# smpurkis/PyTorch-Face-Detection-from-Scratch

Measured on AMD Instinct MI355X. Metric: train imgs/sec (PoolResnet 480^2, bs=256 per GPU), higher is better.
Workload: dtype f32 (3x3 convs: bf16x3 split MFMA, fp32 accumulate)

## Files before the change

pytorch-face-detection-from-scratch_amd/csrc/fdet_ps.hip:

```cpp
#include "fdet_ps.h"

using namespace fdet;

namespace {

__global__ void __launch_bounds__(256)
k_ps_from_f32(const float* __restrict__ x, ps_bf16x8* __restrict__ ps, PsGeo g, PsStrips st, int total) {
  const int t = blockIdx.x * 256 + threadIdx.x;
  if (t >= total) return;
  const int xx = t % st.Wf, r = t / st.Wf;
  const int y = r % g.H, r2 = r / g.H;
  const int gr = r2 % g.C8, n = r2 / g.C8;
  const size_t HW = (size_t)g.H * st.Wf;
  const float* src = x + ((size_t)n * g.C + gr * 8) * HW + (size_t)y * st.Wf + xx;
  ps_bf16x8 hi, lo;
#pragma unroll
  for (int j = 0; j < 8; ++j) {
    const float f = src[j * HW];
    const __bf16 h = (__bf16)f;
    hi[j] = h;
    lo[j] = (__bf16)(f - (float)h);
  }
  const int sidx = xx / st.Ws, xs = xx - sidx * st.Ws;
  const size_t u = (size_t)(sidx * st.Nimg + n) * g.img + (size_t)(gr * g.HP + y) * g.WP + xs + 1;
  ps[u] = hi;
  ps[u + g.plane] = lo;
  if (xs == 0 && sidx > 0) {
    const size_t v = u - (size_t)st.Nimg * g.img + st.Ws;
    ps[v] = hi;
    ps[v + g.plane] = lo;
  }
  if (xs == st.Ws - 1 && sidx + 1 < st.S) {
    const size_t v = u + (size_t)st.Nimg * g.img - st.Ws;
    ps[v] = hi;
    ps[v + g.plane] = lo;
  }
}

__global__ void __launch_bounds__(256)
k_ps_halo(ps_bf16x8* __restrict__ ps, PsGeo g, PsStrips st, int planes, int mode, int total) {
  const int t = blockIdx.x * 256 + threadIdx.x;
  if (t >= total) return;
  const int y = t % g.H;
  int r = t / g.H;
  const int gr = r % g.C8; r /= g.C8;
  const int pl = r % planes; r /= planes;
  const int n = r % st.Nimg, e = r / st.Nimg;
  const size_t row = (size_t)pl * g.plane + (size_t)(gr * g.HP + y) * g.WP;
  const size_t left = (size_t)(e * st.Nimg + n) * g.img + row, right = left + (size_t)st.Nimg * g.img;
  if (mode == 0) {
    ps[left + st.Ws + 1] = ps[right + 1];
    ps[right] = ps[left + st.Ws];
  } else {
    const ps_bf16x8 z = {};
    ps[left + st.Ws + 1] = z;
    ps[right] = z;
  }
}

__global__ void __launch_bounds__(256)
k_ps_to_f32(const ps_bf16x8* __restrict__ ps, float* __restrict__ x, PsGeo g, PsStrips st, int total) {
  const int t = blockIdx.x * 256 + threadIdx.x;
  if (t >= total) return;
  const int xx = t % st.Wf, r = t / st.Wf;
  const int y = r % g.H, r2 = r / g.H;
  const int gr = r2 % g.C8, n = r2 / g.C8;
  const size_t HW = (size_t)g.H * st.Wf;
  const int sidx = xx / st.Ws, xs = xx - sidx * st.Ws;
  const size_t u = (size_t)(sidx * st.Nimg + n) * g.img + (size_t)(gr * g.HP + y) * g.WP + xs + 1;
  const ps_bf16x8 hi = ps[u], lo = ps[u + g.plane];
  float* dst = x + ((size_t)n * g.C + gr * 8) * HW + (size_t)y * st.Wf + xx;
#pragma unroll
  for (int j = 0; j < 8; ++j) dst[j * HW] = (float)hi[j] + (float)lo[j];
}

template <bool P16>
__global__ void __launch_bounds__(256)
k_pool_route_bwd_ps(const float* __restrict__ dout, const unsigned char* __restrict__ route8, const float* __restrict__ scale,
                    ps_bf16x8* __restrict__ dz, PsGeo g, PsStrips st, int Hp, int Wp, float slope, int total) {
  const int t = blockIdx.x * 256 + threadIdx.x;
  if (t >= total) return;
  const int xg = t % Wp, r = t / Wp;
  const int yp = r % Hp, r2 = r / Hp;
  const int gr = r2 % g.C8, n = r2 / g.C8;
  const size_t HWp = (size_t)Hp * Wp;
  const float* src = dout + ((size_t)n * g.C + gr * 8) * HWp + (size_t)yp * Wp + xg;
  const int wsp = st.Ws >> 1, sidx = xg / wsp, xp = xg - sidx * wsp, ns = sidx * st.Nimg + n;
  typedef unsigned u32x2 __attribute__((ext_vector_type(2)));
  const u32x2 rb = *reinterpret_cast<const u32x2*>(route8 + (((size_t)(ns * g.C8 + gr) * Hp + yp) * (g.W >> 1) + xp) * 8);
  float gv[8];
  unsigned mk[8];
#pragma unroll
  for (int j = 0; j < 8; ++j) {
    gv[j] = src[j * HWp] * (scale ? scale[n * g.C + gr * 8 + j] : 1.f);
    mk[j] = (rb[j >> 2] >> (8 * (j & 3))) & 0xffu;
  }
#pragma unroll
  for (int k = 0; k < 4; ++k) {
    ps_bf16x8 hi, lo;
#pragma unroll
    for (int j = 0; j < 8; ++j) {
      const float f = ((int)((mk[j] >> 4) & 3) == k) ? gv[j] * (((mk[j] >> k) & 1) ? 1.f : slope) : 0.f;
      const __bf16 h = (__bf16)f;
      hi[j] = h;
      if (!P16) lo[j] = (__bf16)(f - (float)h);
    }
    const size_t u = (size_t)ns * g.img + (size_t)(gr * g.HP + 2 * yp + (k >> 1)) * g.WP + 2 * xp + (k & 1) + 1;
    dz[u] = hi;
    if (!P16) dz[u + g.plane] = lo;
  }
  if (st.S > 1) {
    const ps_bf16x8 zero = {};
    const bool left = xp == 0 && sidx > 0, right = xp == wsp - 1 && sidx + 1 < st.S;
    if (left || right) {
#pragma unroll
      for (int rr = 0; rr < 2; ++rr) {
        const size_t row = (size_t)ns * g.img + (size_t)(gr * g.HP + 2 * yp + rr) * g.WP;
        if (left) { dz[row] = zero; if (!P16) dz[row + g.plane] = zero; }
        if (right) { dz[row + st.Ws + 1] = zero; if (!P16) dz[row + st.Ws + 1 + g.plane] = zero; }
      }
    }
  }
}

}

namespace {
int pool_route_bwd_ps_run(const float* dout_pooled, const unsigned char* route8, const float* drop_scale,
                          void* dz2_ps, int N, int C, int H, int W, float slope, void* stream, bool p16) {
  PsGeo g;
  PsStrips sp;
  FDET_REQUIRE(dout_pooled && route8 && dz2_ps && !(H & 1) && !(W & 1) && ps_geo_strips(N, C, H, W, g, sp),
               "pool_route_bwd_ps: unsupported shape N=%d C=%d H=%d W=%d (even H, W; C %% 8 == 0)", N, C, H, W);
  const long long total = (long long)N * g.C8 * (H / 2) * (W / 2);
  FDET_REQUIRE(total < (1ll << 31), "pool_route_bwd_ps: tensor too large");
  if (p16)
    hipLaunchKernelGGL(k_pool_route_bwd_ps<true>, dim3((unsigned)((total + 255) / 256)), dim3(256), 0, (hipStream_t)stream,
                       dout_pooled, route8, drop_scale, reinterpret_cast<ps_bf16x8*>(dz2_ps), g, sp, H / 2, W / 2, slope, (int)total);
  else
    hipLaunchKernelGGL(k_pool_route_bwd_ps<false>, dim3((unsigned)((total + 255) / 256)), dim3(256), 0, (hipStream_t)stream,
                       dout_pooled, route8, drop_scale, reinterpret_cast<ps_bf16x8*>(dz2_ps), g, sp, H / 2, W / 2, slope, (int)total);
  return check_launch("fdet_pool_route_bwd_ps");
}
}

extern "C" int fdet_pool_route_bwd_ps(const float* dout_pooled, const unsigned char* route8, const float* drop_scale,
                                      void* dz2_ps, int N, int C, int H, int W, float slope, void* stream) {
  return pool_route_bwd_ps_run(dout_pooled, route8, drop_scale, dz2_ps, N, C, H, W, slope, stream, false);
}
extern "C" int fdet_pool_route_bwd_ps_p16(const float* dout_pooled, const unsigned char* route8, const float* drop_scale,
                                          void* dz2_ps, int N, int C, int H, int W, float slope, void* stream) {
  return pool_route_bwd_ps_run(dout_pooled, route8, drop_scale, dz2_ps, N, C, H, W, slope, stream, true);
}

extern "C" size_t fdet_ps_bytes(int N, int C, int H, int W) {
  PsGeo g;
  PsStrips sp;
  if (!ps_geo_strips(N, C, H, W, g, sp)) return 0;
  return (size_t)(g.N + 2) * g.img * 16;
}

extern "C" size_t fdet_ps_image0_offset(int N, int C, int H, int W) {
  PsGeo g;
  PsStrips sp;
  if (!ps_geo_strips(N, C, H, W, g, sp)) return 0;
  return (size_t)g.img * 16;
}

extern "C" int fdet_ps_strips(int W) {
  PsGeo g;
  PsStrips sp;
  return ps_geo_strips(1, 8, 2, W, g, sp) ? sp.S : 0;
}

extern "C" int fdet_ps_halo_exchange(void* ps, int N, int C, int H, int W, int zero_only, int hi_only, void* stream) {
  PsGeo g;
  PsStrips sp;
  FDET_REQUIRE(ps && ps_geo_strips(N, C, H, W, g, sp), "ps_halo_exchange: unsupported shape N=%d C=%d H=%d W=%d", N, C, H, W);
  if (sp.S == 1) return FDET_OK;
  const int planes = hi_only ? 1 : 2;
  const long long total = (long long)(sp.S - 1) * N * planes * g.C8 * H;
  FDET_REQUIRE(total < (1ll << 31), "ps_halo_exchange: tensor too large");
  hipLaunchKernelGGL(k_ps_halo, dim3((unsigned)((total + 255) / 256)), dim3(256), 0, (hipStream_t)stream,
                     reinterpret_cast<ps_bf16x8*>(ps), g, sp, planes, zero_only ? 1 : 0, (int)total);
  return check_launch("fdet_ps_halo_exchange");
}

extern "C" int fdet_ps_from_f32(const float* x, void* ps, int N, int C, int H, int W, void* stream) {
  PsGeo g;
  PsStrips sp;
  FDET_REQUIRE(x && ps && ps_geo_strips(N, C, H, W, g, sp), "ps_from_f32: unsupported shape N=%d C=%d H=%d W=%d", N, C, H, W);
  const long long total = (long long)N * g.C8 * H * W;
  FDET_REQUIRE(total < (1ll << 31), "ps_from_f32: tensor too large");
  hipLaunchKernelGGL(k_ps_from_f32, dim3((unsigned)((total + 255) / 256)), dim3(256), 0, (hipStream_t)stream, x,
                     reinterpret_cast<ps_bf16x8*>(ps), g, sp, (int)total);
  return check_launch("fdet_ps_from_f32");
}

extern "C" int fdet_ps_to_f32(const void* ps, float* x, int N, int C, int H, int W, void* stream) {
  PsGeo g;
  PsStrips sp;
  FDET_REQUIRE(x && ps && ps_geo_strips(N, C, H, W, g, sp), "ps_to_f32: unsupported shape N=%d C=%d H=%d W=%d", N, C, H, W);
  const long long total = (long long)N * g.C8 * H * W;
  FDET_REQUIRE(total < (1ll << 31), "ps_to_f32: tensor too large");
  hipLaunchKernelGGL(k_ps_to_f32, dim3((unsigned)((total + 255) / 256)), dim3(256), 0, (hipStream_t)stream,
                     reinterpret_cast<const ps_bf16x8*>(ps), x, g, sp, (int)total);
  return check_launch("fdet_ps_to_f32");
}
```

Baseline: 91520.

## Remap pool-route backward to one wavefront per padded output row

```diff
diff --git a/pytorch-face-detection-from-scratch_amd/csrc/fdet_ps.hip b/pytorch-face-detection-from-scratch_amd/csrc/fdet_ps.hip
--- a/pytorch-face-detection-from-scratch_amd/csrc/fdet_ps.hip
+++ b/pytorch-face-detection-from-scratch_amd/csrc/fdet_ps.hip
@@ -74,18 +74,21 @@
   for (int j = 0; j < 8; ++j) dst[j * HW] = (float)hi[j] + (float)lo[j];
 }
 
-template <bool P16>
+template <int WPT, bool P16>
 __global__ void __launch_bounds__(256)
 k_pool_route_bwd_ps(const float* __restrict__ dout, const unsigned char* __restrict__ route8, const float* __restrict__ scale,
-                    ps_bf16x8* __restrict__ dz, PsGeo g, PsStrips st, int Hp, int Wp, float slope, int total) {
-  const int t = blockIdx.x * 256 + threadIdx.x;
-  if (t >= total) return;
-  const int xg = t % Wp, r = t / Wp;
-  const int yp = r % Hp, r2 = r / Hp;
-  const int gr = r2 % g.C8, n = r2 / g.C8;
+                    ps_bf16x8* __restrict__ dz, PsGeo g, PsStrips st, int Hp, int Wp, float slope, int rows) {
+  const int lane = threadIdx.x & 63;
+  const int row = __builtin_amdgcn_readfirstlane((int)(blockIdx.x * 4 + (threadIdx.x >> 6)));
+  if (row >= rows || (WPT == 16 && lane >= 32)) return;
+  const int yp = row % Hp, r2 = row / Hp;
+  const int gr = r2 % g.C8, ns = r2 / g.C8;
+  const int sidx = ns / st.Nimg, n = ns - sidx * st.Nimg;
+  const int s = lane & (WPT - 1), x = s - 1;
+  const bool real = s >= 1 && s <= (sidx == st.S - 1 ? st.Wlast : st.Ws);
+  const int xp = real ? x >> 1 : 0, cp = x & 1;
   const size_t HWp = (size_t)Hp * Wp;
-  const float* src = dout + ((size_t)n * g.C + gr * 8) * HWp + (size_t)yp * Wp + xg;
-  const int wsp = st.Ws >> 1, sidx = xg / wsp, xp = xg - sidx * wsp, ns = sidx * st.Nimg + n;
+  const float* src = dout + ((size_t)n * g.C + gr * 8) * HWp + (size_t)yp * Wp + sidx * (st.Ws >> 1) + xp;
   typedef unsigned u32x2 __attribute__((ext_vector_type(2)));
   const u32x2 rb = *reinterpret_cast<const u32x2*>(route8 + (((size_t)(ns * g.C8 + gr) * Hp + yp) * (g.W >> 1) + xp) * 8);
   float gv[8];
@@ -96,50 +99,53 @@
     mk[j] = (rb[j >> 2] >> (8 * (j & 3))) & 0xffu;
   }
 #pragma unroll
-  for (int k = 0; k < 4; ++k) {
-    ps_bf16x8 hi, lo;
-#pragma unroll
-    for (int j = 0; j < 8; ++j) {
-      const float f = ((int)((mk[j] >> 4) & 3) == k) ? gv[j] * (((mk[j] >> k) & 1) ? 1.f : slope) : 0.f;
-      const __bf16 h = (__bf16)f;
-      hi[j] = h;
-      if (!P16) lo[j] = (__bf16)(f - (float)h);
+  for (int rr = 0; rr < (WPT == 64 ? 2 : 1); ++rr) {
+    const int r = WPT == 64 ? rr : lane / WPT, k = 2 * r + cp;
+    ps_bf16x8 hi = {}, lo = {};
+    if (real) {
+#pragma unroll
+      for (int j = 0; j < 8; ++j) {
+        const float f = ((int)((mk[j] >> 4) & 3) == k) ? gv[j] * (((mk[j] >> k) & 1) ? 1.f : slope) : 0.f;
+        const __bf16 h = (__bf16)f;
+        hi[j] = h;
+        if (!P16) lo[j] = (__bf16)(f - (float)h);
+      }
     }
-    const size_t u = (size_t)ns * g.img + (size_t)(gr * g.HP + 2 * yp + (k >> 1)) * g.WP + 2 * xp + (k & 1) + 1;
+    const size_t u = (size_t)ns * g.img + (size_t)(gr * g.HP + 2 * yp + r) * g.WP + s;
     dz[u] = hi;
     if (!P16) dz[u + g.plane] = lo;
   }
-  if (st.S > 1) {
-    const ps_bf16x8 zero = {};
-    const bool left = xp == 0 && sidx > 0, right = xp == wsp - 1 && sidx + 1 < st.S;
-    if (left || right) {
-#pragma unroll
-      for (int rr = 0; rr < 2; ++rr) {
-        const size_t row = (size_t)ns * g.img + (size_t)(gr * g.HP + 2 * yp + rr) * g.WP;
-        if (left) { dz[row] = zero; if (!P16) dz[row + g.plane] = zero; }
-        if (right) { dz[row + st.Ws + 1] = zero; if (!P16) dz[row + st.Ws + 1 + g.plane] = zero; }
-      }
-    }
-  }
 }
 
 }
 
 namespace {
+template <int WPT>
+void pool_route_bwd_ps_launch(const float* dout_pooled, const unsigned char* route8, const float* drop_scale, void* dz2_ps,
+                              const PsGeo& g, const PsStrips& sp, int Hp, int Wp, float slope, int rows, void* stream, bool p16) {
+  const dim3 grid((unsigned)((rows + 3) / 4));
+  if (p16)
+    hipLaunchKernelGGL((k_pool_route_bwd_ps<WPT, true>), grid, dim3(256), 0, (hipStream_t)stream,
+                       dout_pooled, route8, drop_scale, reinterpret_cast<ps_bf16x8*>(dz2_ps), g, sp, Hp, Wp, slope, rows);
+  else
+    hipLaunchKernelGGL((k_pool_route_bwd_ps<WPT, false>), grid, dim3(256), 0, (hipStream_t)stream,
+                       dout_pooled, route8, drop_scale, reinterpret_cast<ps_bf16x8*>(dz2_ps), g, sp, Hp, Wp, slope, rows);
+}
+
 int pool_route_bwd_ps_run(const float* dout_pooled, const unsigned char* route8, const float* drop_scale,
                           void* dz2_ps, int N, int C, int H, int W, float slope, void* stream, bool p16) {
   PsGeo g;
   PsStrips sp;
   FDET_REQUIRE(dout_pooled && route8 && dz2_ps && !(H & 1) && !(W & 1) && ps_geo_strips(N, C, H, W, g, sp),
                "pool_route_bwd_ps: unsupported shape N=%d C=%d H=%d W=%d (even H, W; C %% 8 == 0)", N, C, H, W);
-  const long long total = (long long)N * g.C8 * (H / 2) * (W / 2);
-  FDET_REQUIRE(total < (1ll << 31), "pool_route_bwd_ps: tensor too large");
-  if (p16)
-    hipLaunchKernelGGL(k_pool_route_bwd_ps<true>, dim3((unsigned)((total + 255) / 256)), dim3(256), 0, (hipStream_t)stream,
-                       dout_pooled, route8, drop_scale, reinterpret_cast<ps_bf16x8*>(dz2_ps), g, sp, H / 2, W / 2, slope, (int)total);
+  const long long rows = (long long)g.N * g.C8 * (H / 2);
+  FDET_REQUIRE(rows * 64 < (1ll << 31), "pool_route_bwd_ps: tensor too large");
+  if (g.WP == 64)
+    pool_route_bwd_ps_launch<64>(dout_pooled, route8, drop_scale, dz2_ps, g, sp, H / 2, W / 2, slope, (int)rows, stream, p16);
+  else if (g.WP == 32)
+    pool_route_bwd_ps_launch<32>(dout_pooled, route8, drop_scale, dz2_ps, g, sp, H / 2, W / 2, slope, (int)rows, stream, p16);
   else
-    hipLaunchKernelGGL(k_pool_route_bwd_ps<false>, dim3((unsigned)((total + 255) / 256)), dim3(256), 0, (hipStream_t)stream,
-                       dout_pooled, route8, drop_scale, reinterpret_cast<ps_bf16x8*>(dz2_ps), g, sp, H / 2, W / 2, slope, (int)total);
+    pool_route_bwd_ps_launch<16>(dout_pooled, route8, drop_scale, dz2_ps, g, sp, H / 2, W / 2, slope, (int)rows, stream, p16);
   return check_launch("fdet_pool_route_bwd_ps");
 }
 }
```

Result: no change. 92020 (median of 6 runs) (+0.5%).
